# AI-Unicamp/interspeech_ser

Measured on AMD Instinct MI355X. Metric: utterances/sec (10 s @16 kHz) WavLM-large embed extract, higher is better.
Workload: dtype bf16; 1 GPU; microsoft/wavlm-large embed extract, batch=16 x 10 s @16 kHz per GPU, all 25 hidden states to HBM, mode=bf16; a counted step = 8 such batches (128 utterances per GPU), 2 in flight at a time; batch=16, batches_in_flight=2, frames_per_utt=499, parallelism=utterance-sharded x1, no collective (one process)

## Files before the change

interspeech_ser_amd/csrc/gemm.hip:

```cpp
#include "ser_common.h"
#include "launch_plan.h"
#ifndef SER_GEMM_PP
#define SER_GEMM_PP 27
#endif
#include <stdlib.h>
#include <stdio.h>
#include <utility>
#ifdef SER_GEMM_DBG
extern "C" { void* ser_gemm_dbg_ptr = nullptr; }
__device__ unsigned long long* ser_gemm_dbg_dev = nullptr;
#endif

typedef const __attribute__((address_space(1))) void* gptr_t;
typedef __attribute__((address_space(3))) void* lptr_t;

__device__ __forceinline__ const char* uniform_ptr(const void* p) {
    const uint64_t v = (uint64_t)p;
    const uint32_t lo = __builtin_amdgcn_readfirstlane((uint32_t)v), hi = __builtin_amdgcn_readfirstlane((uint32_t)(v >> 32));
    return (const char*)(((uint64_t)hi << 32) | lo);
}
template <int BYTES>
__device__ __forceinline__ void dma_lds(const void* ubase, uint32_t voff, uint32_t lds_addr) {
    static_assert(BYTES == 16 || BYTES == 4, "dwordx4 or dword");
    if constexpr (BYTES == 16)
        asm volatile("s_mov_b32 m0, %2\n\tglobal_load_lds_dwordx4 %0, %1" :: "v"(voff), "s"(ubase), "s"(lds_addr) : "memory");
    else
        asm volatile("s_mov_b32 m0, %2\n\tglobal_load_lds_dword %0, %1" :: "v"(voff), "s"(ubase), "s"(lds_addr) : "memory");
}

template <int N>
__device__ __forceinline__ void wait_vmcnt() {
    if constexpr (N == 0) asm volatile("s_waitcnt vmcnt(0)" ::: "memory");
    else if constexpr (N == 1) asm volatile("s_waitcnt vmcnt(1)" ::: "memory");
    else if constexpr (N == 2) asm volatile("s_waitcnt vmcnt(2)" ::: "memory");
    else if constexpr (N == 3) asm volatile("s_waitcnt vmcnt(3)" ::: "memory");
    else if constexpr (N == 4) asm volatile("s_waitcnt vmcnt(4)" ::: "memory");
    else if constexpr (N == 5) asm volatile("s_waitcnt vmcnt(5)" ::: "memory");
    else if constexpr (N == 6) asm volatile("s_waitcnt vmcnt(6)" ::: "memory");
    else if constexpr (N == 7) asm volatile("s_waitcnt vmcnt(7)" ::: "memory");
    else if constexpr (N == 8) asm volatile("s_waitcnt vmcnt(8)" ::: "memory");
    else if constexpr (N == 10) asm volatile("s_waitcnt vmcnt(10)" ::: "memory");
    else if constexpr (N == 12) asm volatile("s_waitcnt vmcnt(12)" ::: "memory");
    else if constexpr (N == 16) asm volatile("s_waitcnt vmcnt(16)" ::: "memory");
    else static_assert(N < 0, "add a case");
}

__device__ __forceinline__ void mfma_scale8(f32x4& acc, const i32x8& a, const i32x8& b, int sa, int sb) {
    asm volatile("v_mfma_scale_f32_16x16x128_f8f6f4 %0, %1, %2, %0, %3, %4 op_sel_hi:[0,0,0]" : "+v"(acc) : "v"(a), "v"(b), "v"(sa), "v"(sb));
}
__device__ __forceinline__ void mfma_scale_drain() {
    asm volatile("s_nop 15\n\ts_nop 15\n\ts_nop 7" ::: "memory");
}

template <int WM, int WN, int TM, int TN, int BK, int ST, int MODE, bool LNEPI, int OM = MODE>
__global__ __launch_bounds__(64 * WM * WN, 2)
void ser_gemm_kernel(const ser_gemm_args p) {
    constexpr int NW = WM * WN, NT = 64 * NW;
    constexpr int BM = WM * TM * 16, BN = WN * TN * 16;
    constexpr int CH = BK / 8;
    constexpr int ROWB = BK * 2;
    constexpr int RPP = 1024 / ROWB;
    constexpr bool M16 = (MODE == SER_MODE_FP16M);
    constexpr int NPL = M16 ? 1 : mode_traits<MODE>::planes;
    constexpr int A_BYTES = BM * ROWB, W_BYTES = BN * ROWB, STAGE = NPL * (A_BYTES + W_BYTES);
    static_assert(!M16 || (BK == 64 && !LNEPI && (BM + BN) % 64 == 0), "FP16M: 64-deep K tiles, dense epilogue");
    constexpr int SCW = BM + BN;
    constexpr int LA = BM / RPP / NW, LW = BN / RPP / NW;
    constexpr int LPT = NPL * (LA + LW);
    constexpr int KS = BK / 32;
    static_assert(BM % (RPP * NW) == 0 && BN % (RPP * NW) == 0, "tile/wave mismatch");
    extern __shared__ __attribute__((aligned(16))) char lds[];

    const int tid = threadIdx.x;
    const int lane = tid & 63;
    const int wave = __builtin_amdgcn_readfirstlane(tid >> 6);
    const int wm = wave / WN, wn = wave % WN;
#ifdef SER_GEMM_DBG
    const unsigned long long dbg_e0 = __builtin_amdgcn_s_memtime();
#endif

    const int ntn = (p.N + BN - 1) / BN;
    const int ntm = (p.M + BM - 1) / BM;
    int bid = blockIdx.x;
    {
        const int nwg = ntm * ntn;
        const int q = nwg >> 3, r = nwg & 7, xcd = bid & 7;
        const int base = (xcd < r) ? xcd * (q + 1) : r * (q + 1) + (xcd - r) * q;
        bid = base + (bid >> 3);
    }
    const int mt = bid / ntn;
    const int nt = bid - mt * ntn;
    const int g = blockIdx.y;
    const int m0 = mt * BM, n0 = nt * BN;

    const unsigned short* Abase = (const unsigned short*)p.A + (int64_t)g * p.a_group_stride;
    const unsigned short* Wbase = (const unsigned short*)p.W + (int64_t)g * p.w_group_stride;

    const int prow = lane / CH, ppos = lane % CH;
    uint32_t aoff[LA], woff[LW];
    const int m0c = m0 < p.M ? m0 : p.M - 1;
    const int64_t arow0 = p.a_rowoff ? (int64_t)p.a_rowoff[m0c] * 8 : (int64_t)m0c * p.lda;
    const char* const Atile = uniform_ptr(Abase + arow0);
    const char* const Wtile = uniform_ptr(Wbase + (int64_t)n0 * p.K);
#pragma unroll
    for (int q = 0; q < LA; ++q) {
        const int R = (q * NW + wave) * RPP + prow;
        const int f = (BK == 64) ? (R & 7) : ((R >> 1) & 3);
        const int c = ppos ^ f;
        int m = m0 + R;
        m = m < p.M ? m : p.M - 1;
        const int64_t arow = p.a_rowoff ? (int64_t)p.a_rowoff[m] * 8 : (int64_t)m * p.lda;
        aoff[q] = (uint32_t)((arow - arow0 + c * 8) * 2);
    }
#pragma unroll
    for (int q = 0; q < LW; ++q) {
        const int R = (q * NW + wave) * RPP + prow;
        const int f = (BK == 64) ? (R & 7) : ((R >> 1) & 3);
        const int c = ppos ^ f;
        int n = n0 + R;
        n = n < p.N ? n : p.N - 1;
        woff[q] = (uint32_t)(((int64_t)(n - n0) * p.K + c * 8) * 2);
    }
    const uint32_t lds0 = __builtin_amdgcn_readfirstlane((uint32_t)(uintptr_t)(__attribute__((address_space(3))) char*)lds);

    const int nk = p.K / BK;
    const int total = M16 ? 2 * nk : nk;
    const int tpc = p.kc ? p.kc / BK : 0x7fffffff;

    unsigned char* const scl = (unsigned char*)(lds + ST * STAGE + (LNEPI ? 0 : BM * 8));
    const int sc_chunk = M16 ? (wave % (SCW / 64)) : 0;
    const bool sc_is_a = sc_chunk * 64 < BM;
    const char* const sc_base = uniform_ptr(sc_is_a ? p.a_scale : p.w_scale);
    const int64_t sc_step = (sc_is_a ? p.a_scale_ld : p.w_scale_ld) * 4;
    uint32_t sc_off = 0;
    if constexpr (M16) {
        const int r = sc_chunk * 64 + lane;
        int i = sc_is_a ? m0 + r : n0 + r - BM;
        const int lim = sc_is_a ? p.M : p.N;
        i = i < lim ? i : lim - 1;
        sc_off = (uint32_t)i * 4u;
    }
    int i_kk = 0, i_cc = 0, i_cj = 0, i_stage = 0;
    const char* is_ua = nullptr; const char* is_uw = nullptr;
    uint32_t is_dstA = 0, is_dstW = 0;
    auto issue_begin = [&]() {
        int64_t koffA = (int64_t)i_cj * p.ldj + (int64_t)i_cc * BK;
        int64_t koffW = (int64_t)i_kk * BK;
        if constexpr (M16) {
            koffA = (int64_t)(i_kk >> 1) * BK + (i_kk & 1) * p.a_plane_stride;
            koffW = (int64_t)(i_kk >> 1) * BK + (i_kk & 1) * p.w_plane_stride;
            if (i_kk & 1) dma_lds<4>(sc_base + (int64_t)(i_kk >> 1) * sc_step, sc_off, lds0 + (uint32_t)(ST * STAGE + (LNEPI ? 0 : BM * 8) + (i_stage * SCW + sc_chunk * 64) * 4));
        }
        is_dstA = lds0 + i_stage * STAGE + wave * 1024;
        is_dstW = is_dstA + NPL * A_BYTES;
        is_ua = Atile + koffA * 2;
        is_uw = Wtile + koffW * 2;
    };
    auto issue_piece = [&](int j) {
        const int pl = j / (LA + LW), q = j % (LA + LW);
        if (q < LA) dma_lds<16>(is_ua + (int64_t)pl * p.a_plane_stride * 2, aoff[q < LA ? q : 0], is_dstA + pl * A_BYTES + q * NW * 1024);
        else dma_lds<16>(is_uw + (int64_t)pl * p.w_plane_stride * 2, woff[q >= LA ? q - LA : 0], is_dstW + pl * W_BYTES + (q - LA) * NW * 1024);
    };
    auto issue_end = [&]() {
        ++i_kk; ++i_cc;
        if (i_cc == tpc) { i_cc = 0; ++i_cj; }
        i_stage = (i_stage + 1 == ST) ? 0 : i_stage + 1;
    };
    auto issue = [&]() {
        issue_begin();
#pragma unroll
        for (int j = 0; j < LPT; ++j) issue_piece(j);
        issue_end();
    };

    f32x4 acc[TN][TM];
#pragma unroll
    for (int a = 0; a < TN; ++a)
#pragma unroll
        for (int b = 0; b < TM; ++b) acc[a][b] = (f32x4){0.f, 0.f, 0.f, 0.f};

    const int frow = lane & 15, fq = lane >> 4;
    const int fsw = (BK == 64) ? (lane & 7) : ((frow >> 1) & 3);
    int offA[KS], offW[KS];
#pragma unroll
    for (int s = 0; s < KS; ++s) {
        const int phys = ((s * 4 + fq) ^ fsw) << 4;
        offA[s] = (wm * TM * 16 + frow) * ROWB + phys;
        offW[s] = NPL * A_BYTES + (wn * TN * 16 + frow) * ROWB + phys;
    }

    constexpr int CPL = TN * 4;
    const int ncol0 = n0 + wn * (TN * 16) + fq * 4;
    const int64_t gcol = (int64_t)g * p.c_group_stride + ncol0;
    float bias[CPL], csum[CPL];
    auto load_cols = [&]() {
#pragma unroll
        for (int j = 0; j < CPL; ++j) { bias[j] = 0.f; csum[j] = 0.f; }
        if (p.bias) {
#pragma unroll
            for (int j4 = 0; j4 < TN; ++j4)
                if (ncol0 + j4 * 16 < p.N) {
                    const f32x4 b = *(const f32x4*)(p.bias + (int64_t)g * p.N + ncol0 + j4 * 16);
                    bias[j4 * 4 + 0] = b[0]; bias[j4 * 4 + 1] = b[1]; bias[j4 * 4 + 2] = b[2]; bias[j4 * 4 + 3] = b[3];
                }
        }
        if (p.ln_colsum) {
#pragma unroll
            for (int j4 = 0; j4 < TN; ++j4)
                if (ncol0 + j4 * 16 < p.N) {
                    const f32x4 b = *(const f32x4*)(p.ln_colsum + ncol0 + j4 * 16);
                    csum[j4 * 4 + 0] = b[0]; csum[j4 * 4 + 1] = b[1]; csum[j4 * 4 + 2] = b[2]; csum[j4 * 4 + 3] = b[3];
                }
        }
    };
    constexpr bool LATE_COLS = M16;
    if constexpr (!LATE_COLS) load_cols();

#pragma unroll
    for (int t = 0; t < ST - 1; ++t)
        if (t < total) issue();

    float* lnst = (float*)(lds + ST * STAGE);
    if (p.ln_stats_in) {
        for (int r = tid; r < BM; r += NT) {
            int m = m0 + r;
            m = m < p.M ? m : p.M - 1;
            const float* ps = p.ln_stats_in + (int64_t)m * p.ln_groups * 2;
            f32x4 pv[16];
#pragma unroll
            for (int u = 0; u < 16; ++u)
                pv[u] = (2 * u < p.ln_groups) ? *(const f32x4*)(ps + 4 * u) : (f32x4){0.f, 0.f, 0.f, 0.f};
            float s1 = 0.f, s2 = 0.f;
#pragma unroll
            for (int u = 0; u < 16; ++u) { s1 += pv[u][0] + pv[u][2]; s2 += pv[u][1] + pv[u][3]; }
            const float invK = 1.0f / (float)p.K;
            const float mu = s1 * invK;
            const float var = fmaxf(s2 * invK - mu * mu, 0.f);
            lnst[2 * r] = mu;
            lnst[2 * r + 1] = rsqrtf(var + p.ln_eps);
            if (p.mean_out && nt == 0 && g == 0 && m0 + r < p.M) p.mean_out[m] = mu + (p.ln_shift ? p.ln_shift[m] : 0.f);
            if (p.lnstat_out && nt == 0 && g == 0 && m0 + r < p.M) *(f32x2*)(p.lnstat_out + 2 * (int64_t)m) = (f32x2){mu, lnst[2 * r + 1]};
        }
        __syncthreads();
    }

#ifdef SER_GEMM_DBG
    const unsigned long long dbg_t0 = __builtin_amdgcn_s_memtime(), dbg_r0 = __builtin_amdgcn_s_memrealtime();
#endif
    constexpr int PP_BIT = NPL == 2 ? (LNEPI ? 16 : 8) : (LNEPI ? 4 : (TM * TN >= 32 ? 1 : 2));
    constexpr bool PP = !M16 && (SER_GEMM_PP & PP_BIT) && NW == 8 && (KS == 2 || NPL == 2);
    constexpr int PH = (NPL == 1 && TM * TN >= 32) ? KS : 1;
    constexpr int SPP = KS / PH;
    constexpr bool PPW = PP && NPL == 2 && KS == 1 && TN >= 8;
    if constexpr (PPW) {
        constexpr int TNH = TN / 2;
        const int late = wave >> 2;
        if (total >= ST - 1) wait_vmcnt<LPT * (ST - 2)>(); else wait_vmcnt<0>();
        __builtin_amdgcn_s_barrier();
        __builtin_amdgcn_sched_barrier(0);
        if (late) __builtin_amdgcn_s_barrier();
        int stage = 0;
        for (int kt = 0; kt < total; ++kt) {
            const bool more = kt + ST - 1 < total;
            if (more) issue();
            const char* sb = lds + stage * STAGE;
            stage = (stage + 1 == ST) ? 0 : stage + 1;
            const bool last = kt + 1 == total;
            bf16x8 ah[TM], al[TM];
#pragma unroll
            for (int ph = 0; ph < 2; ++ph) {
                bf16x8 wh[TNH], wl[TNH];
                if (ph == 0) {
#pragma unroll
                    for (int x = 0; x < TM; ++x) {
                        ah[x] = *(const bf16x8*)(sb + offA[0] + x * 16 * ROWB);
                        al[x] = *(const bf16x8*)(sb + offA[0] + A_BYTES + x * 16 * ROWB);
                    }
                }
#pragma unroll
                for (int x = 0; x < TNH; ++x) {
                    wh[x] = *(const bf16x8*)(sb + offW[0] + (ph * TNH + x) * 16 * ROWB);
                    wl[x] = *(const bf16x8*)(sb + offW[0] + W_BYTES + (ph * TNH + x) * 16 * ROWB);
                }
                asm volatile("s_waitcnt lgkmcnt(0)" ::: "memory");
                if (ph == 1 && late) { if (more) wait_vmcnt<LPT * (ST - 2)>(); else wait_vmcnt<0>(); }
                __builtin_amdgcn_sched_barrier(0);
                __builtin_amdgcn_s_barrier();
                __builtin_amdgcn_sched_barrier(0);
                __builtin_amdgcn_s_setprio(1);
#pragma unroll
                for (int nj = 0; nj < TNH; ++nj)
#pragma unroll
                    for (int mi = 0; mi < TM; ++mi) {
                        const int ni = ph * TNH + nj;
                        acc[ni][mi] = mfma16<MODE>(wl[nj], ah[mi], acc[ni][mi]);
                        acc[ni][mi] = mfma16<MODE>(wh[nj], al[mi], acc[ni][mi]);
                        acc[ni][mi] = mfma16<MODE>(wh[nj], ah[mi], acc[ni][mi]);
                    }
                __builtin_amdgcn_s_setprio(0);
                if (ph == 1 && !late) { if (more) wait_vmcnt<LPT * (ST - 2)>(); else wait_vmcnt<0>(); }
                __builtin_amdgcn_sched_barrier(0);
                if (!(ph == 1 && last && late)) __builtin_amdgcn_s_barrier();
                __builtin_amdgcn_sched_barrier(0);
            }
        }
    }
    if constexpr (PP && !PPW) {
        const int late = wave >> 2;
        if (total >= ST - 1) wait_vmcnt<LPT * (ST - 2)>(); else wait_vmcnt<0>();
        __builtin_amdgcn_s_barrier();
        __builtin_amdgcn_sched_barrier(0);
        if (late) __builtin_amdgcn_s_barrier();
        int stage = 0;
        for (int kt = 0; kt < total; ++kt) {
            const bool more = kt + ST - 1 < total;
            if (more) issue();
            const char* sb = lds + stage * STAGE;
            stage = (stage + 1 == ST) ? 0 : stage + 1;
            const bool last = kt + 1 == total;
#pragma unroll
            for (int ph = 0; ph < PH; ++ph) {
                bf16x8 af[SPP][TM], wf[SPP][TN];
                bf16x8 al[NPL == 2 ? SPP : 1][NPL == 2 ? TM : 1], wl[NPL == 2 ? SPP : 1][NPL == 2 ? TN : 1];
#pragma unroll
                for (int u = 0; u < SPP; ++u) {
#pragma unroll
                    for (int x = 0; x < TM; ++x) {
                        af[u][x] = *(const bf16x8*)(sb + offA[ph * SPP + u] + x * 16 * ROWB);
                        if constexpr (NPL == 2) al[u][x] = *(const bf16x8*)(sb + offA[ph * SPP + u] + A_BYTES + x * 16 * ROWB);
                    }
#pragma unroll
                    for (int x = 0; x < TN; ++x) {
                        wf[u][x] = *(const bf16x8*)(sb + offW[ph * SPP + u] + x * 16 * ROWB);
                        if constexpr (NPL == 2) wl[u][x] = *(const bf16x8*)(sb + offW[ph * SPP + u] + W_BYTES + x * 16 * ROWB);
                    }
                }
                asm volatile("s_waitcnt lgkmcnt(0)" ::: "memory");
                if (ph == PH - 1 && late) { if (more) wait_vmcnt<LPT * (ST - 2)>(); else wait_vmcnt<0>(); }
                __builtin_amdgcn_sched_barrier(0);
                __builtin_amdgcn_s_barrier();
                __builtin_amdgcn_sched_barrier(0);
                __builtin_amdgcn_s_setprio(1);
#pragma unroll
                for (int u = 0; u < SPP; ++u)
#pragma unroll
                    for (int ni = 0; ni < TN; ++ni)
#pragma unroll
                        for (int mi = 0; mi < TM; ++mi) {
                            if constexpr (NPL == 2) {
                                acc[ni][mi] = mfma16<MODE>(wl[u][ni], af[u][mi], acc[ni][mi]);
                                acc[ni][mi] = mfma16<MODE>(wf[u][ni], al[u][mi], acc[ni][mi]);
                                acc[ni][mi] = mfma16<MODE>(wf[u][ni], af[u][mi], acc[ni][mi]);
                            } else {
                                acc[ni][mi] = mfma16<MODE>(wf[u][ni], af[u][mi], acc[ni][mi]);
                            }
                        }
                __builtin_amdgcn_s_setprio(0);
                if (ph == PH - 1 && !late) { if (more) wait_vmcnt<LPT * (ST - 2)>(); else wait_vmcnt<0>(); }
                __builtin_amdgcn_sched_barrier(0);
                if (!(ph == PH - 1 && last && late)) __builtin_amdgcn_s_barrier();
                __builtin_amdgcn_sched_barrier(0);
            }
        }
    }

    if constexpr (M16) {
        constexpr int LPTH = LPT, LPTE = LPT + 1;
        constexpr bool PPM = (NW == 8);
        constexpr int PHM = (TM * TN >= 32) ? 2 : 1;
        constexpr int SPM = KS / PHM;
        constexpr int PHE = PHM;
        constexpr int TMP = TM / PHE;
        auto wait_landed = [&](bool more, int young) {
            if (!more || ST == 2) wait_vmcnt<0>();
            else if (young & 1) wait_vmcnt<LPTE * (ST - 2)>();
            else wait_vmcnt<LPTH * (ST - 2)>();
        };
        auto h_phase_reads = [&](const char* sb, int ph, auto& af, auto& wf) {
#pragma unroll
            for (int u = 0; u < SPM; ++u) {
#pragma unroll
                for (int x = 0; x < TM; ++x) af[u][x] = *(const bf16x8*)(sb + offA[ph * SPM + u] + x * 16 * ROWB);
#pragma unroll
                for (int x = 0; x < TN; ++x) wf[u][x] = *(const bf16x8*)(sb + offW[ph * SPM + u] + x * 16 * ROWB);
            }
        };
        auto h_phase_mfma = [&](auto& af, auto& wf) {
#pragma unroll
            for (int u = 0; u < SPM; ++u)
#pragma unroll
                for (int ni = 0; ni < TN; ++ni)
#pragma unroll
                    for (int mi = 0; mi < TM; ++mi) acc[ni][mi] = mfma16<SER_MODE_FP16>(wf[u][ni], af[u][mi], acc[ni][mi]);
        };
        auto e_phase_reads = [&](const char* sb, const unsigned char* scb, int ph, auto& a8, auto& w8, auto& sa, auto& sw) {
#pragma unroll
            for (int x = 0; x < TMP; ++x) {
                const int mi = ph * TMP + x;
                const u32x4 c0 = *(const u32x4*)(sb + offA[0] + mi * 16 * ROWB), c1 = *(const u32x4*)(sb + offA[1] + mi * 16 * ROWB);
                a8[x] = (i32x8){(int)c0[0], (int)c0[1], (int)c0[2], (int)c0[3], (int)c1[0], (int)c1[1], (int)c1[2], (int)c1[3]};
                sa[x] = scb[(wm * TM * 16 + mi * 16 + frow) * 4 + fq];
            }
#pragma unroll
            for (int x = 0; x < TN; ++x) {
                const u32x4 c0 = *(const u32x4*)(sb + offW[0] + x * 16 * ROWB), c1 = *(const u32x4*)(sb + offW[1] + x * 16 * ROWB);
                w8[x] = (i32x8){(int)c0[0], (int)c0[1], (int)c0[2], (int)c0[3], (int)c1[0], (int)c1[1], (int)c1[2], (int)c1[3]};
                sw[x] = scb[(BM + wn * TN * 16 + x * 16 + frow) * 4 + fq];
            }
        };
        auto e_phase_mfma = [&](int ph, auto& a8, auto& w8, auto& sa, auto& sw) {
#pragma unroll
            for (int ni = 0; ni < TN; ++ni)
#pragma unroll
                for (int x = 0; x < TMP; ++x)
                    mfma_scale8(acc[ni][ph * TMP + x], w8[ni], a8[x], sw[ni], sa[x]);
        };
        if constexpr (PPM) {
            const int late = wave >> 2;
            wait_landed(total >= ST - 1, ST - 2);
            __builtin_amdgcn_s_barrier();
            __builtin_amdgcn_sched_barrier(0);
            if (late) __builtin_amdgcn_s_barrier();
            int stage = 0;
            auto unit = [&](int kt, auto etag) {
                constexpr bool EU = decltype(etag)::value;
                const bool more = kt + ST - 1 < total;
#ifdef SER_GEMM_DBG
                unsigned long long stp[8] = {0, 0, 0, 0, 0, 0, 0, 0};
                const bool stamp = ser_gemm_dbg_dev && blockIdx.x == 40 && lane == 0 && kt >= 8 && kt < 16;
#define SER_STAMP(i) do { __builtin_amdgcn_sched_barrier(0); if (stamp) stp[i] = __builtin_amdgcn_s_memtime(); __builtin_amdgcn_sched_barrier(0); } while (0)
                SER_STAMP(0);
#else
#define SER_STAMP(i) do { } while (0)
#endif
                SER_STAMP(1);
                const char* sb = lds + stage * STAGE;
                const unsigned char* scb = scl + stage * SCW * 4;
                stage = (stage + 1 == ST) ? 0 : stage + 1;
                const bool last = kt + 1 == total;
                constexpr int NPH = EU ? PHE : PHM;
#pragma unroll
                for (int ph = 0; ph < NPH; ++ph) {
                    bf16x8 af[EU ? 1 : SPM][EU ? 1 : TM], wf[EU ? 1 : SPM][EU ? 1 : TN];
                    i32x8 a8[EU ? TMP : 1], w8[EU ? TN : 1];
                    int sa[EU ? TMP : 1], sw[EU ? TN : 1];
                    if constexpr (!EU) h_phase_reads(sb, ph, af, wf);
                    else e_phase_reads(sb, scb, ph, a8, w8, sa, sw);
                    if (ph == 0 && more) { __builtin_amdgcn_sched_barrier(0); issue(); }
                    asm volatile("s_waitcnt lgkmcnt(0)" ::: "memory");
                    if (ph == 0) SER_STAMP(2);
                    if (ph == NPH - 1 && late) wait_landed(more, kt + ST - 1);
                    if (ph == 0) SER_STAMP(3);
                    __builtin_amdgcn_sched_barrier(0);
                    __builtin_amdgcn_s_barrier();
                    __builtin_amdgcn_sched_barrier(0);
                    if (ph == 0) SER_STAMP(4);
                    __builtin_amdgcn_s_setprio(1);
                    if constexpr (!EU) h_phase_mfma(af, wf);
                    else e_phase_mfma(ph, a8, w8, sa, sw);
                    __builtin_amdgcn_s_setprio(0);
                    if (ph == 0) SER_STAMP(5);
                    if (ph == NPH - 1 && !late) wait_landed(more, kt + ST - 1);
                    if (ph == 0) SER_STAMP(6);
                    __builtin_amdgcn_sched_barrier(0);
                    if (!(ph == NPH - 1 && last && late)) __builtin_amdgcn_s_barrier();
                    __builtin_amdgcn_sched_barrier(0);
                    if (ph == 0) SER_STAMP(7);
                }
#ifdef SER_GEMM_DBG
                if (stamp) for (int i = 0; i < 8; ++i) ser_gemm_dbg_dev[262144 + ((wave * 8 + (kt - 8)) * 8 + i)] = stp[i];
#endif
            };
            for (int kt = 0; kt < total; kt += 2) {
                unit(kt, std::false_type{});
                unit(kt + 1, std::true_type{});
            }
        } else {
            int stage = 0;
            auto unit = [&](int kt, auto etag) {
                constexpr bool EU = decltype(etag)::value;
                wait_landed(kt + (ST - 2) < total, kt + ST - 2);
                __builtin_amdgcn_s_barrier();
                if (kt + ST - 1 < total) issue();
                const char* sb = lds + stage * STAGE;
                const unsigned char* scb = scl + stage * SCW * 4;
                stage = (stage + 1 == ST) ? 0 : stage + 1;
#pragma unroll
                for (int ph = 0; ph < (EU ? PHE : PHM); ++ph) {
                    if constexpr (!EU) {
                        bf16x8 af[SPM][TM], wf[SPM][TN];
                        h_phase_reads(sb, ph, af, wf);
                        __builtin_amdgcn_s_setprio(1);
                        h_phase_mfma(af, wf);
                        __builtin_amdgcn_s_setprio(0);
                    } else {
                        i32x8 a8[TMP], w8[TN];
                        int sa[TMP], sw[TN];
                        e_phase_reads(sb, scb, ph, a8, w8, sa, sw);
                        __builtin_amdgcn_s_setprio(1);
                        e_phase_mfma(ph, a8, w8, sa, sw);
                        __builtin_amdgcn_s_setprio(0);
                    }
                }
            };
            for (int kt = 0; kt < total; kt += 2) {
                unit(kt, std::false_type{});
                unit(kt + 1, std::true_type{});
            }
        }
    }
    if constexpr (M16) mfma_scale_drain();
    int c_stage = 0;
    for (int kt = 0; kt < ((PP || M16) ? 0 : total); ++kt) {
        if (kt + (ST - 2) < total) wait_vmcnt<LPT * (ST - 2)>();
        else wait_vmcnt<0>();
        __builtin_amdgcn_s_barrier();
        if (kt + ST - 1 < total) issue();
        const char* sb = lds + c_stage * STAGE;
        c_stage = (c_stage + 1 == ST) ? 0 : c_stage + 1;
        if constexpr (NPL == 1) {
            constexpr bool PIPE = (TM * TN * 4 + KS * (TM + TN) * 4) <= 208;
            bf16x8 af[KS][TM], wf[KS][TN];
            if constexpr (PIPE) {
#pragma unroll
                for (int s = 0; s < KS; ++s) {
#pragma unroll
                    for (int x = 0; x < TM; ++x) af[s][x] = *(const bf16x8*)(sb + offA[s] + x * 16 * ROWB);
#pragma unroll
                    for (int x = 0; x < TN; ++x) wf[s][x] = *(const bf16x8*)(sb + offW[s] + x * 16 * ROWB);
                }
            }
#pragma unroll
            for (int s = 0; s < KS; ++s) {
                if constexpr (!PIPE) {
#pragma unroll
                    for (int x = 0; x < TM; ++x) af[s][x] = *(const bf16x8*)(sb + offA[s] + x * 16 * ROWB);
#pragma unroll
                    for (int x = 0; x < TN; ++x) wf[s][x] = *(const bf16x8*)(sb + offW[s] + x * 16 * ROWB);
                }
                __builtin_amdgcn_s_setprio(1);
#pragma unroll
                for (int ni = 0; ni < TN; ++ni)
#pragma unroll
                    for (int mi = 0; mi < TM; ++mi)
                        acc[ni][mi] = mfma16<MODE>(wf[s][ni], af[s][mi], acc[ni][mi]);
                __builtin_amdgcn_s_setprio(0);
            }
        } else {
#pragma unroll
            for (int s = 0; s < KS; ++s) {
                bf16x8 ah[TM], al[TM], wh[TN], wl[TN];
#pragma unroll
                for (int x = 0; x < TM; ++x) {
                    ah[x] = *(const bf16x8*)(sb + offA[s] + x * 16 * ROWB);
                    al[x] = *(const bf16x8*)(sb + offA[s] + A_BYTES + x * 16 * ROWB);
                }
#pragma unroll
                for (int x = 0; x < TN; ++x) {
                    wh[x] = *(const bf16x8*)(sb + offW[s] + x * 16 * ROWB);
                    wl[x] = *(const bf16x8*)(sb + offW[s] + W_BYTES + x * 16 * ROWB);
                }
                __builtin_amdgcn_s_setprio(1);
#pragma unroll
                for (int ni = 0; ni < TN; ++ni)
#pragma unroll
                    for (int mi = 0; mi < TM; ++mi) {
                        acc[ni][mi] = mfma16<MODE>(wl[ni], ah[mi], acc[ni][mi]);
                        acc[ni][mi] = mfma16<MODE>(wh[ni], al[mi], acc[ni][mi]);
                        acc[ni][mi] = mfma16<MODE>(wh[ni], ah[mi], acc[ni][mi]);
                    }
                __builtin_amdgcn_s_setprio(0);
            }
        }
    }

#ifdef SER_GEMM_DBG
    {
        __builtin_amdgcn_sched_barrier(0);
        const unsigned long long t1 = __builtin_amdgcn_s_memtime(), r1 = __builtin_amdgcn_s_memrealtime();
        unsigned long long* d = ser_gemm_dbg_dev;
        if (d && wave == 0 && lane == 0 && blockIdx.y == 0) {
            d[blockIdx.x * 2] = t1 - dbg_t0; d[blockIdx.x * 2 + 1] = r1 - dbg_r0;
            d[131072 + blockIdx.x * 4] = dbg_t0 - dbg_e0; d[131072 + blockIdx.x * 4 + 1] = t1;
        }
    }
#endif
    if constexpr (LATE_COLS) load_cols();
    float ramax = 0.f;
    if constexpr (LNEPI) {
        __syncthreads();
        float* red = (float*)lds;
        const float invN = 1.0f / (float)p.N;
        float mean[TM], rstd[TM], nmr[TM];
#pragma unroll
        for (int mi = 0; mi < TM; ++mi) {
            float s1 = 0.f, s2 = 0.f;
#pragma unroll
            for (int ni = 0; ni < TN; ++ni)
#pragma unroll
                for (int r = 0; r < 4; ++r) {
                    const float x = acc[ni][mi][r] + bias[ni * 4 + r];
                    acc[ni][mi][r] = x;
                    if (ncol0 + ni * 16 < p.N) { s1 += x; s2 += x * x; }
                }
            s1 += __shfl_xor(s1, 16, 64); s2 += __shfl_xor(s2, 16, 64);
            s1 += __shfl_xor(s1, 32, 64); s2 += __shfl_xor(s2, 32, 64);
            if (fq == 0) {
                red[((wm * TM * 16 + mi * 16 + frow) * WN + wn) * 2] = s1;
                red[((wm * TM * 16 + mi * 16 + frow) * WN + wn) * 2 + 1] = s2;
            }
        }
        __syncthreads();
#pragma unroll
        for (int mi = 0; mi < TM; ++mi) {
            float s1 = 0.f, s2 = 0.f;
#pragma unroll
            for (int w = 0; w < WN; ++w) {
                s1 += red[((wm * TM * 16 + mi * 16 + frow) * WN + w) * 2];
                s2 += red[((wm * TM * 16 + mi * 16 + frow) * WN + w) * 2 + 1];
            }
            mean[mi] = s1 * invN;
            rstd[mi] = rsqrtf(fmaxf(s2 * invN - mean[mi] * mean[mi], 0.f) + p.ln_eps);
            nmr[mi] = -mean[mi] * rstd[mi];
        }
        float lg[CPL], lb[CPL];
#pragma unroll
        for (int j4 = 0; j4 < TN; ++j4) {
            f32x4 a = {0.f, 0.f, 0.f, 0.f}, b = {0.f, 0.f, 0.f, 0.f};
            if (ncol0 + j4 * 16 < p.N) {
                a = *(const f32x4*)(p.ln_gamma + ncol0 + j4 * 16);
                b = *(const f32x4*)(p.ln_beta + ncol0 + j4 * 16);
            }
#pragma unroll
            for (int r = 0; r < 4; ++r) { lg[j4 * 4 + r] = a[r]; lb[j4 * 4 + r] = b[r]; }
        }
#pragma unroll
        for (int mi = 0; mi < TM; ++mi) {
            const int m = m0 + wm * TM * 16 + mi * 16 + frow;
            if (m >= p.M) continue;
            const int64_t orow = p.out_rowmap ? (int64_t)p.out_rowmap[m] : (int64_t)m;
#pragma unroll
            for (int ni = 0; ni < TN; ni += 2) {
                const bool ok0 = ncol0 + ni * 16 < p.N, ok1 = ncol0 + ni * 16 + 16 < p.N;
                float v[8];
#pragma unroll
                for (int r = 0; r < 8; ++r) {
                    const int nj = ni + (r >> 2), rr = r & 3;
                    v[r] = fmaf(fmaf(acc[nj][mi][rr], rstd[mi], nmr[mi]), lg[nj * 4 + rr], lb[nj * 4 + rr]);
                }
                if (p.act == SER_ACT_GELU) {
#pragma unroll
                    for (int r = 0; r < 8; r += 2) {
                        const f32x2 y = gelu2<MODE == SER_MODE_BF16>((f32x2){v[r], v[r + 1]});
                        v[r] = y[0]; v[r + 1] = y[1];
                    }
                }
                if (p.out_f32) {
                    f32x4 o0 = {v[0], v[1], v[2], v[3]}, o1 = {v[4], v[5], v[6], v[7]};
                    if (ok0) *(f32x4*)(p.out_f32 + (int64_t)m * p.ldo_f32 + gcol + ni * 16) = o0;
                    if (ok1) *(f32x4*)(p.out_f32 + (int64_t)m * p.ldo_f32 + gcol + ni * 16 + 16) = o1;
                }
                if (p.out_act) {
                    const int c8 = ni * 16 + ((fq & 1) ? 12 : 0);
                    store_act8_swap<MODE>((unsigned short*)p.out_act + orow * p.ldo_act + gcol + c8, p.out_plane_stride,
                                          ncol0 + c8 < p.N, v);
                    if constexpr (mode_traits<MODE>::f16) {
                        if (p.range_flag) range_fold8(ramax, v, ok0, ok1);
                    }
                }
            }
        }
    } else {
        const bool do_scale = p.col_scale_end > 0;
        const bool do_stat = p.stat_out != nullptr;
        float cs[TM];
#pragma unroll
        for (int mi = 0; mi < TM; ++mi) {
            cs[mi] = 0.f;
            if (p.shift_out) {
                int m = m0 + wm * TM * 16 + mi * 16 + frow;
                m = m < p.M ? m : p.M - 1;
                cs[mi] = p.shift_const + (p.shift_in ? p.shift_in[m] : 0.f);
            }
        }
        constexpr int RB = (TM * TN > 16) ? 2 : (TM < 4 ? TM : 4);
        f32x4 rres[RB][TN];
#pragma unroll
        for (int mi = 0; mi < TM; ++mi) {
            if (mi % RB == 0 && p.residual) {
#pragma unroll
                for (int u = 0; u < RB; ++u) {
                    int mr = m0 + wm * TM * 16 + (mi + u) * 16 + frow;
                    mr = mr < p.M ? mr : p.M - 1;
                    const int rr_ = p.res_row_mod ? (mr % p.res_row_mod) : mr;
#pragma unroll
                    for (int ni = 0; ni < TN; ++ni) {
                        f32x4 r = {0.f, 0.f, 0.f, 0.f};
                        if (ncol0 + ni * 16 < p.N) r = *(const f32x4*)(p.residual + (int64_t)rr_ * p.ldr + gcol + ni * 16);
                        rres[u][ni] = r;
                    }
                }
            }
            const int m = m0 + wm * TM * 16 + mi * 16 + frow;
            if (m >= p.M) continue;
            const int64_t orow = p.out_rowmap ? (int64_t)p.out_rowmap[m] : (int64_t)m;
            float mu = 0.f, rs = 1.f;
            if (p.ln_stats_in) {
                mu = lnst[2 * (wm * TM * 16 + mi * 16 + frow)];
                rs = lnst[2 * (wm * TM * 16 + mi * 16 + frow) + 1];
            }
            const float cshift = cs[mi];
            if (p.shift_out && nt == 0 && g == 0 && wn == 0 && fq == 0) p.shift_out[m] = cshift;
            const float* gsc = nullptr;
            const float* gsh = nullptr;
            if (p.gn_scale) {
                int lo = 0, hi = p.gn_B;
                while (hi - lo > 1) { const int mid = (lo + hi) >> 1; if (p.gn_row_offs[mid] <= m) lo = mid; else hi = mid; }
                gsc = p.gn_scale + (int64_t)lo * p.gn_ld + ncol0;
                gsh = p.gn_shift + (int64_t)lo * p.gn_ld + ncol0;
            }
            float st1 = 0.f, st2 = 0.f;
            unsigned mcode[2] = {0u, 0u};
#pragma unroll
            for (int ni = 0; ni < TN; ni += 2) {
                const bool ok0 = ncol0 + ni * 16 < p.N, ok1 = ncol0 + ni * 16 + 16 < p.N;
                float v[8];
#pragma unroll
                for (int r = 0; r < 8; ++r) {
                    const int nj = ni + (r >> 2), rr = r & 3;
                    float x = fmaf(rs, acc[nj][mi][rr] - mu * csum[nj * 4 + rr], bias[nj * 4 + rr]);
                    if (gsc && ncol0 + nj * 16 < p.N) x = fmaf(x, gsc[nj * 16 + rr], gsh[nj * 16 + rr]);
                    if (do_scale && ncol0 + nj * 16 < p.col_scale_end) x *= p.col_scale;
                    v[r] = x;
                }
                if (p.act == SER_ACT_GELU) {
#pragma unroll
                    for (int r = 0; r < 8; r += 2) {
                        const f32x2 y = gelu2<MODE == SER_MODE_BF16>((f32x2){v[r], v[r + 1]});
                        v[r] = y[0]; v[r + 1] = y[1];
                    }
                }
                if (p.residual) {
                    const f32x4 r0 = rres[mi % RB][ni], r1 = rres[mi % RB][ni + 1];
                    v[0] += r0[0]; v[1] += r0[1]; v[2] += r0[2]; v[3] += r0[3];
                    v[4] += r1[0]; v[5] += r1[1]; v[6] += r1[2]; v[7] += r1[3];
                }
                if (p.out_f32) {
                    float* op = p.out_f32 + (int64_t)m * p.ldo_f32 + gcol + ni * 16 - p.f32_col_begin;
                    f32x4 o0 = {v[0], v[1], v[2], v[3]}, o1 = {v[4], v[5], v[6], v[7]};
                    if (ok0 && ncol0 + ni * 16 >= p.f32_col_begin) *(f32x4*)op = o0;
                    if (ok1 && ncol0 + ni * 16 + 16 >= p.f32_col_begin) *(f32x4*)(op + 16) = o1;
                }
                if (p.shift_out) {
#pragma unroll
                    for (int r = 0; r < 8; ++r) v[r] -= cshift;
                }
                if (do_stat && ok0) {
#pragma unroll
                    for (int r = 0; r < 4; ++r) { st1 += v[r]; st2 += v[r] * v[r]; }
                }
                if (do_stat && ok1) {
#pragma unroll
                    for (int r = 4; r < 8; ++r) { st1 += v[r]; st2 += v[r] * v[r]; }
                }
                if (p.out_act) {
                    const int c8 = ni * 16 + ((fq & 1) ? 12 : 0);
                    if constexpr (OM == SER_MODE_FP16M) {
                        store_act8_swap<SER_MODE_FP16>((unsigned short*)p.out_act + orow * p.ldo_act + gcol + c8, 0, ncol0 + c8 < p.N, v);
                        float lo[8], ax = 0.f, al = 0.f;
#pragma unroll
                        for (int r = 0; r < 8; r += 2) {
                            const unsigned h2 = pack_h2(v[r], v[r + 1]);
                            lo[r] = v[r] - h2f((unsigned short)(h2 & 0xffffu));
                            lo[r + 1] = v[r + 1] - h2f((unsigned short)(h2 >> 16));
                            ax = fmaxf(ax, fmaxf(fabsf(v[r]), fabsf(v[r + 1])));
                            al = fmaxf(al, fmaxf(fabsf(lo[r]), fabsf(lo[r + 1])));
                        }
                        if (p.range_flag) range_fold8(ramax, v, ok0, ok1);
                        ax = max_rowquad(ax); al = max_rowquad(al);
                        const unsigned cx = mx_code(ax), cl = mx_code(al);
                        const float ix = mx_inv(cx), il = mx_inv(cl);
                        unsigned q4[4] = {mx_pack4(lo[0] * il, lo[1] * il, lo[2] * il, lo[3] * il), mx_pack4(lo[4] * il, lo[5] * il, lo[6] * il, lo[7] * il),
                                          mx_pack4(v[0] * ix, v[1] * ix, v[2] * ix, v[3] * ix), mx_pack4(v[4] * ix, v[5] * ix, v[6] * ix, v[7] * ix)};
                        transpose_rowquad(q4);
                        const int64_t bcol = gcol - fq * 4 + ni * 16;
                        unsigned char* seg = (unsigned char*)((unsigned short*)p.out_act + p.out_plane_stride) + (orow * p.ldo_act + (bcol & ~(int64_t)63)) * 2;
                        if (ok0) *(u32x4*)(seg + (fq >> 1) * 64 + (bcol & 63) + (fq & 1) * 16) = (u32x4){q4[0], q4[1], q4[2], q4[3]};
                        mcode[(ni >> 1) & 1] = cl | (cx << 16);
                        if (((ni >> 1) & 1) && fq == 0 && ok0)
                            p.out_scale[(bcol >> 6) * p.out_scale_ld + orow] = (mcode[0] & 0xffu) | ((mcode[1] & 0xffu) << 8) | (mcode[0] & 0xff0000u) | ((mcode[1] & 0xff0000u) << 8);
                    } else {
                        store_act8_swap<OM>((unsigned short*)p.out_act + orow * p.ldo_act + gcol + c8, p.out_plane_stride,
                                            ncol0 + c8 < p.N, v);
                        if constexpr (mode_traits<OM>::f16) {
                            if (p.range_flag) range_fold8(ramax, v, ok0, ok1);
                        }
                    }
                }
            }
            if (p.stat_out) {
                st1 += __shfl_xor(st1, 16, 64); st2 += __shfl_xor(st2, 16, 64);
                st1 += __shfl_xor(st1, 32, 64); st2 += __shfl_xor(st2, 32, 64);
                const int cstart = n0 + wn * (TN * 16);
                const int grp = g * ((p.N + 63) >> 6) + (cstart >> 6);
                if (fq == 0 && cstart < p.N && grp < p.stat_groups) {
                    float* d = p.stat_out + ((int64_t)m * p.stat_groups + grp) * 2;
                    d[0] = st1; d[1] = st2;
                    if constexpr (TN * 16 > 64) {
                        if (cstart + 64 < p.N) { d[2] = 0.f; d[3] = 0.f; }
                    }
                }
            }
        }
    }
    if constexpr (mode_traits<OM>::f16) range_report(p.range_flag, ramax);
#ifdef SER_GEMM_DBG
    {
        __builtin_amdgcn_sched_barrier(0);
        asm volatile("s_waitcnt vmcnt(0)" ::: "memory");
        const unsigned long long t2 = __builtin_amdgcn_s_memtime();
        unsigned long long* d = ser_gemm_dbg_dev;
        if (d && wave == 0 && lane == 0 && blockIdx.y == 0) d[131072 + blockIdx.x * 4 + 2] = t2;
    }
#endif
}

template <int... I, class F>
static bool with_index(int i, std::integer_sequence<int, I...>, F&& f) { return ser_with_mode<I...>(i, f); }

template <int TILE, int PAIR>
static int launch_planned(const ser_gemm_args* a, const gemm_launch& pl, hipStream_t s) {
    constexpr gemm_tile t = GEMM_TILE[TILE];
    constexpr gemm_pair pr = GEMM_PAIR[PAIR];
    auto k = ser_gemm_kernel<t.WM, t.WN, t.TM, t.TN, t.BK, t.ST, pr.mode, t.LNEPI, pr.om>;
    static std::atomic<bool> ready{false};
    if (pl.lds > 65536)
        if (hipError_t e = ser_lds_optin(k, pl.lds, ready)) return ser_fail((int)e, "ser_gemm: cannot raise dynamic LDS to %d", pl.lds);
    hipLaunchKernelGGL(k, dim3(pl.grid_x, pl.grid_y, 1), dim3((unsigned)pl.block, 1, 1), pl.lds, s, *a);
    return ser_check_launch("ser_gemm");
}

extern "C" int ser_gemm(const ser_gemm_args* a, void* stream) {
    gemm_launch pl;
    if (int rc = gemm_plan(a, &pl)) return rc;
// ... 20 lines not shown
```

Baseline: 2061 utterances/s.

## Skip dead M-tail fragments in GEMM main loops and epilogues

Computes a per-wave count of live 16-row fragments and, for tail tiles, runs a specialized K-loop that skips LDS reads and MFMAs for rows beyond M. Epilogue, LN-stat and residual loops also break early past the live rows, and LN stat rows past M are filled with defaults instead of clamped reloads. The change targets wasted matrix work in the partial last M tile (frames_per_utt=499 makes M non-aligned). In exchange it doubles the instantiated loop bodies, which costs code size and could raise register pressure, and it is excluded for several configurations through TAIL_RULE.

```diff
diff --git a/interspeech_ser_amd/csrc/gemm.hip b/interspeech_ser_amd/csrc/gemm.hip
--- a/interspeech_ser_amd/csrc/gemm.hip
+++ b/interspeech_ser_amd/csrc/gemm.hip
@@ -50,6 +50,37 @@
 }
 __device__ __forceinline__ void mfma_scale_drain() {
     asm volatile("s_nop 15\n\ts_nop 15\n\ts_nop 7" ::: "memory");
+}
+
+template <int TM, class F>
+__device__ __forceinline__ void frag_rows(bool full, int lv, F&& f) {
+#pragma unroll
+    for (int mi = 0; mi < TM; ++mi) {
+        if (!full && mi >= lv) break;
+        f(mi);
+    }
+}
+template <int TN, int TM, class F>
+__device__ __forceinline__ void frag_pairs(bool full, int lv, F&& f) {
+    if (full) {
+#pragma unroll
+        for (int ni = 0; ni < TN; ++ni)
+#pragma unroll
+            for (int mi = 0; mi < TM; ++mi) f(ni, mi);
+    } else {
+#pragma unroll
+        for (int mi = 0; mi < TM; ++mi) {
+            if (mi >= lv) break;
+#pragma unroll
+            for (int ni = 0; ni < TN; ++ni) f(ni, mi);
+        }
+    }
+}
+template <int TM>
+__device__ __forceinline__ int live_rows(bool full, int live) {
+    if (full) return TM;
+    asm volatile("" : "+s"(live));
+    return live;
 }
 
 template <int WM, int WN, int TM, int TN, int BK, int ST, int MODE, bool LNEPI, int OM = MODE>
@@ -92,6 +123,12 @@
     const int nt = bid - mt * ntn;
     const int g = blockIdx.y;
     const int m0 = mt * BM, n0 = nt * BN;
+    constexpr bool TAIL_RULE = !((NPL == 2 && TN == 8) || (NPL == 1 && LNEPI && WM == 2) || (NPL == 2 && OM == SER_MODE_FP16M) ||
+                                 (NPL == 2 && BK == 64 && MODE == SER_MODE_FP16X && OM == SER_MODE_FP16X) ||
+                                 (MODE == SER_MODE_FP16 && OM == SER_MODE_FP16X && TM * TN == 32));
+    const int live = TAIL_RULE ? __builtin_amdgcn_readfirstlane(max(0, min(TM, (p.M - m0 - wm * TM * 16 + 15) >> 4))) : TM;
+    using full_k = std::true_type;
+    using tail_k = std::false_type;
 
     const unsigned short* Abase = (const unsigned short*)p.A + (int64_t)g * p.a_group_stride;
     const unsigned short* Wbase = (const unsigned short*)p.W + (int64_t)g * p.w_group_stride;
@@ -223,8 +260,8 @@
     float* lnst = (float*)(lds + ST * STAGE);
     if (p.ln_stats_in) {
         for (int r = tid; r < BM; r += NT) {
-            int m = m0 + r;
-            m = m < p.M ? m : p.M - 1;
+            const int m = m0 + r;
+            if (m >= p.M) { lnst[2 * r] = 0.f; lnst[2 * r + 1] = 1.f; continue; }
             const float* ps = p.ln_stats_in + (int64_t)m * p.ln_groups * 2;
             f32x4 pv[16];
 #pragma unroll
@@ -238,8 +275,8 @@
             const float var = fmaxf(s2 * invK - mu * mu, 0.f);
             lnst[2 * r] = mu;
             lnst[2 * r + 1] = rsqrtf(var + p.ln_eps);
-            if (p.mean_out && nt == 0 && g == 0 && m0 + r < p.M) p.mean_out[m] = mu + (p.ln_shift ? p.ln_shift[m] : 0.f);
-            if (p.lnstat_out && nt == 0 && g == 0 && m0 + r < p.M) *(f32x2*)(p.lnstat_out + 2 * (int64_t)m) = (f32x2){mu, lnst[2 * r + 1]};
+            if (p.mean_out && nt == 0 && g == 0) p.mean_out[m] = mu + (p.ln_shift ? p.ln_shift[m] : 0.f);
+            if (p.lnstat_out && nt == 0 && g == 0) *(f32x2*)(p.lnstat_out + 2 * (int64_t)m) = (f32x2){mu, lnst[2 * r + 1]};
         }
         __syncthreads();
     }
@@ -312,6 +349,8 @@
         __builtin_amdgcn_sched_barrier(0);
         if (late) __builtin_amdgcn_s_barrier();
         int stage = 0;
+        auto kloop = [&](auto kform) {
+        constexpr bool FULL = decltype(kform)::value;
         for (int kt = 0; kt < total; ++kt) {
             const bool more = kt + ST - 1 < total;
             if (more) issue();
@@ -320,19 +359,21 @@
             const bool last = kt + 1 == total;
 #pragma unroll
             for (int ph = 0; ph < PH; ++ph) {
+                const int lv = live_rows<TM>(FULL, live);
                 bf16x8 af[SPP][TM], wf[SPP][TN];
                 bf16x8 al[NPL == 2 ? SPP : 1][NPL == 2 ? TM : 1], wl[NPL == 2 ? SPP : 1][NPL == 2 ? TN : 1];
 #pragma unroll
                 for (int u = 0; u < SPP; ++u) {
-#pragma unroll
-                    for (int x = 0; x < TM; ++x) {
+                    frag_rows<TM>(FULL, lv, [&](int x) {
                         af[u][x] = *(const bf16x8*)(sb + offA[ph * SPP + u] + x * 16 * ROWB);
                         if constexpr (NPL == 2) al[u][x] = *(const bf16x8*)(sb + offA[ph * SPP + u] + A_BYTES + x * 16 * ROWB);
-                    }
-#pragma unroll
-                    for (int x = 0; x < TN; ++x) {
-                        wf[u][x] = *(const bf16x8*)(sb + offW[ph * SPP + u] + x * 16 * ROWB);
-                        if constexpr (NPL == 2) wl[u][x] = *(const bf16x8*)(sb + offW[ph * SPP + u] + W_BYTES + x * 16 * ROWB);
+                    });
+                    if (FULL || lv > 0) {
+#pragma unroll
+                        for (int x = 0; x < TN; ++x) {
+                            wf[u][x] = *(const bf16x8*)(sb + offW[ph * SPP + u] + x * 16 * ROWB);
+                            if constexpr (NPL == 2) wl[u][x] = *(const bf16x8*)(sb + offW[ph * SPP + u] + W_BYTES + x * 16 * ROWB);
+                        }
                     }
                 }
                 asm volatile("s_waitcnt lgkmcnt(0)" ::: "memory");
@@ -343,18 +384,15 @@
                 __builtin_amdgcn_s_setprio(1);
 #pragma unroll
                 for (int u = 0; u < SPP; ++u)
-#pragma unroll
-                    for (int ni = 0; ni < TN; ++ni)
-#pragma unroll
-                        for (int mi = 0; mi < TM; ++mi) {
-                            if constexpr (NPL == 2) {
-                                acc[ni][mi] = mfma16<MODE>(wl[u][ni], af[u][mi], acc[ni][mi]);
-                                acc[ni][mi] = mfma16<MODE>(wf[u][ni], al[u][mi], acc[ni][mi]);
-                                acc[ni][mi] = mfma16<MODE>(wf[u][ni], af[u][mi], acc[ni][mi]);
-                            } else {
-                                acc[ni][mi] = mfma16<MODE>(wf[u][ni], af[u][mi], acc[ni][mi]);
-                            }
+                    frag_pairs<TN, TM>(FULL, lv, [&](int ni, int mi) {
+                        if constexpr (NPL == 2) {
+                            acc[ni][mi] = mfma16<MODE>(wl[u][ni], af[u][mi], acc[ni][mi]);
+                            acc[ni][mi] = mfma16<MODE>(wf[u][ni], al[u][mi], acc[ni][mi]);
+                            acc[ni][mi] = mfma16<MODE>(wf[u][ni], af[u][mi], acc[ni][mi]);
+                        } else {
+                            acc[ni][mi] = mfma16<MODE>(wf[u][ni], af[u][mi], acc[ni][mi]);
                         }
+                    });
                 __builtin_amdgcn_s_setprio(0);
                 if (ph == PH - 1 && !late) { if (more) wait_vmcnt<LPT * (ST - 2)>(); else wait_vmcnt<0>(); }
                 __builtin_amdgcn_sched_barrier(0);
@@ -362,6 +400,8 @@
                 __builtin_amdgcn_sched_barrier(0);
             }
         }
+        };
+        if (live == TM) kloop(full_k{}); else kloop(tail_k{});
     }
 
     if constexpr (M16) {
@@ -376,44 +416,50 @@
             else if (young & 1) wait_vmcnt<LPTE * (ST - 2)>();
             else wait_vmcnt<LPTH * (ST - 2)>();
         };
-        auto h_phase_reads = [&](const char* sb, int ph, auto& af, auto& wf) {
+        auto h_phase_reads = [&](const char* sb, int ph, int lv, auto& af, auto& wf) {
 #pragma unroll
             for (int u = 0; u < SPM; ++u) {
 #pragma unroll
-                for (int x = 0; x < TM; ++x) af[u][x] = *(const bf16x8*)(sb + offA[ph * SPM + u] + x * 16 * ROWB);
-#pragma unroll
-                for (int x = 0; x < TN; ++x) wf[u][x] = *(const bf16x8*)(sb + offW[ph * SPM + u] + x * 16 * ROWB);
+                for (int x = 0; x < TM; ++x)
+                    if (x < lv) af[u][x] = *(const bf16x8*)(sb + offA[ph * SPM + u] + x * 16 * ROWB);
+#pragma unroll
+                for (int x = 0; x < TN; ++x)
+                    if (lv > 0) wf[u][x] = *(const bf16x8*)(sb + offW[ph * SPM + u] + x * 16 * ROWB);
             }
         };
-        auto h_phase_mfma = [&](auto& af, auto& wf) {
+        auto h_phase_mfma = [&](int lv, auto& af, auto& wf) {
 #pragma unroll
             for (int u = 0; u < SPM; ++u)
 #pragma unroll
                 for (int ni = 0; ni < TN; ++ni)
 #pragma unroll
-                    for (int mi = 0; mi < TM; ++mi) acc[ni][mi] = mfma16<SER_MODE_FP16>(wf[u][ni], af[u][mi], acc[ni][mi]);
+                    for (int mi = 0; mi < TM; ++mi)
+                        if (mi < lv) acc[ni][mi] = mfma16<SER_MODE_FP16>(wf[u][ni], af[u][mi], acc[ni][mi]);
         };
-        auto e_phase_reads = [&](const char* sb, const unsigned char* scb, int ph, auto& a8, auto& w8, auto& sa, auto& sw) {
+        auto e_phase_reads = [&](const char* sb, const unsigned char* scb, int ph, int lv, auto& a8, auto& w8, auto& sa, auto& sw) {
 #pragma unroll
             for (int x = 0; x < TMP; ++x) {
                 const int mi = ph * TMP + x;
-                const u32x4 c0 = *(const u32x4*)(sb + offA[0] + mi * 16 * ROWB), c1 = *(const u32x4*)(sb + offA[1] + mi * 16 * ROWB);
-                a8[x] = (i32x8){(int)c0[0], (int)c0[1], (int)c0[2], (int)c0[3], (int)c1[0], (int)c1[1], (int)c1[2], (int)c1[3]};
-                sa[x] = scb[(wm * TM * 16 + mi * 16 + frow) * 4 + fq];
-            }
-#pragma unroll
-            for (int x = 0; x < TN; ++x) {
-                const u32x4 c0 = *(const u32x4*)(sb + offW[0] + x * 16 * ROWB), c1 = *(const u32x4*)(sb + offW[1] + x * 16 * ROWB);
-                w8[x] = (i32x8){(int)c0[0], (int)c0[1], (int)c0[2], (int)c0[3], (int)c1[0], (int)c1[1], (int)c1[2], (int)c1[3]};
-                sw[x] = scb[(BM + wn * TN * 16 + x * 16 + frow) * 4 + fq];
-            }
+                if (mi < lv) {
+                    const u32x4 c0 = *(const u32x4*)(sb + offA[0] + mi * 16 * ROWB), c1 = *(const u32x4*)(sb + offA[1] + mi * 16 * ROWB);
+                    a8[x] = (i32x8){(int)c0[0], (int)c0[1], (int)c0[2], (int)c0[3], (int)c1[0], (int)c1[1], (int)c1[2], (int)c1[3]};
+                    sa[x] = scb[(wm * TM * 16 + mi * 16 + frow) * 4 + fq];
+                }
+            }
+#pragma unroll
+            for (int x = 0; x < TN; ++x)
+                if (ph * TMP < lv) {
+                    const u32x4 c0 = *(const u32x4*)(sb + offW[0] + x * 16 * ROWB), c1 = *(const u32x4*)(sb + offW[1] + x * 16 * ROWB);
+                    w8[x] = (i32x8){(int)c0[0], (int)c0[1], (int)c0[2], (int)c0[3], (int)c1[0], (int)c1[1], (int)c1[2], (int)c1[3]};
+                    sw[x] = scb[(BM + wn * TN * 16 + x * 16 + frow) * 4 + fq];
+                }
         };
-        auto e_phase_mfma = [&](int ph, auto& a8, auto& w8, auto& sa, auto& sw) {
+        auto e_phase_mfma = [&](int ph, int lv, auto& a8, auto& w8, auto& sa, auto& sw) {
 #pragma unroll
             for (int ni = 0; ni < TN; ++ni)
 #pragma unroll
                 for (int x = 0; x < TMP; ++x)
-                    mfma_scale8(acc[ni][ph * TMP + x], w8[ni], a8[x], sw[ni], sa[x]);
+                    if (ph * TMP + x < lv) mfma_scale8(acc[ni][ph * TMP + x], w8[ni], a8[x], sw[ni], sa[x]);
         };
         if constexpr (PPM) {
             const int late = wave >> 2;
@@ -422,8 +468,9 @@
             __builtin_amdgcn_sched_barrier(0);
             if (late) __builtin_amdgcn_s_barrier();
             int stage = 0;
-            auto unit = [&](int kt, auto etag) {
+            auto unit = [&](int kt, auto etag, auto kform) {
                 constexpr bool EU = decltype(etag)::value;
+                const int lv = live_rows<TM>(decltype(kform)::value, live);
                 const bool more = kt + ST - 1 < total;
 #ifdef SER_GEMM_DBG
                 unsigned long long stp[8] = {0, 0, 0, 0, 0, 0, 0, 0};
@@ -444,8 +491,8 @@
                     bf16x8 af[EU ? 1 : SPM][EU ? 1 : TM], wf[EU ? 1 : SPM][EU ? 1 : TN];
                     i32x8 a8[EU ? TMP : 1], w8[EU ? TN : 1];
                     int sa[EU ? TMP : 1], sw[EU ? TN : 1];
-                    if constexpr (!EU) h_phase_reads(sb, ph, af, wf);
-                    else e_phase_reads(sb, scb, ph, a8, w8, sa, sw);
+                    if constexpr (!EU) h_phase_reads(sb, ph, lv, af, wf);
+                    else e_phase_reads(sb, scb, ph, lv, a8, w8, sa, sw);
                     if (ph == 0 && more) { __builtin_amdgcn_sched_barrier(0); issue(); }
                     asm volatile("s_waitcnt lgkmcnt(0)" ::: "memory");
                     if (ph == 0) SER_STAMP(2);
@@ -456,8 +503,8 @@
                     __builtin_amdgcn_sched_barrier(0);
                     if (ph == 0) SER_STAMP(4);
                     __builtin_amdgcn_s_setprio(1);
-                    if constexpr (!EU) h_phase_mfma(af, wf);
-                    else e_phase_mfma(ph, a8, w8, sa, sw);
+                    if constexpr (!EU) h_phase_mfma(lv, af, wf);
+                    else e_phase_mfma(ph, lv, a8, w8, sa, sw);
                     __builtin_amdgcn_s_setprio(0);
                     if (ph == 0) SER_STAMP(5);
                     if (ph == NPH - 1 && !late) wait_landed(more, kt + ST - 1);
@@ -471,14 +518,18 @@
                 if (stamp) for (int i = 0; i < 8; ++i) ser_gemm_dbg_dev[262144 + ((wave * 8 + (kt - 8)) * 8 + i)] = stp[i];
 #endif
             };
-            for (int kt = 0; kt < total; kt += 2) {
-                unit(kt, std::false_type{});
-                unit(kt + 1, std::true_type{});
-            }
+            auto kloop = [&](auto kform) {
+                for (int kt = 0; kt < total; kt += 2) {
+                    unit(kt, std::false_type{}, kform);
+                    unit(kt + 1, std::true_type{}, kform);
+                }
+            };
+            if (live == TM) kloop(full_k{}); else kloop(tail_k{});
         } else {
             int stage = 0;
-            auto unit = [&](int kt, auto etag) {
+            auto unit = [&](int kt, auto etag, auto kform) {
                 constexpr bool EU = decltype(etag)::value;
+                const int lv = live_rows<TM>(decltype(kform)::value, live);
                 wait_landed(kt + (ST - 2) < total, kt + ST - 2);
                 __builtin_amdgcn_s_barrier();
                 if (kt + ST - 1 < total) issue();
@@ -489,29 +540,35 @@
                 for (int ph = 0; ph < (EU ? PHE : PHM); ++ph) {
                     if constexpr (!EU) {
                         bf16x8 af[SPM][TM], wf[SPM][TN];
-                        h_phase_reads(sb, ph, af, wf);
+                        h_phase_reads(sb, ph, lv, af, wf);
                         __builtin_amdgcn_s_setprio(1);
-                        h_phase_mfma(af, wf);
+                        h_phase_mfma(lv, af, wf);
                         __builtin_amdgcn_s_setprio(0);
                     } else {
                         i32x8 a8[TMP], w8[TN];
                         int sa[TMP], sw[TN];
-                        e_phase_reads(sb, scb, ph, a8, w8, sa, sw);
+                        e_phase_reads(sb, scb, ph, lv, a8, w8, sa, sw);
                         __builtin_amdgcn_s_setprio(1);
-                        e_phase_mfma(ph, a8, w8, sa, sw);
+                        e_phase_mfma(ph, lv, a8, w8, sa, sw);
                         __builtin_amdgcn_s_setprio(0);
                     }
                 }
             };
-            for (int kt = 0; kt < total; kt += 2) {
-                unit(kt, std::false_type{});
-                unit(kt + 1, std::true_type{});
-            }
+            auto kloop = [&](auto kform) {
+                for (int kt = 0; kt < total; kt += 2) {
+                    unit(kt, std::false_type{}, kform);
+                    unit(kt + 1, std::true_type{}, kform);
+                }
+            };
+            if (live == TM) kloop(full_k{}); else kloop(tail_k{});
         }
     }
     if constexpr (M16) mfma_scale_drain();
     int c_stage = 0;
+    auto ring = [&](auto kform) {
+    constexpr bool FULL = decltype(kform)::value;
     for (int kt = 0; kt < ((PP || M16) ? 0 : total); ++kt) {
+        const int lv = live_rows<TM>(FULL, live);
         if (kt + (ST - 2) < total) wait_vmcnt<LPT * (ST - 2)>();
         else wait_vmcnt<0>();
         __builtin_amdgcn_s_barrier();
@@ -525,25 +582,25 @@
 #pragma unroll
                 for (int s = 0; s < KS; ++s) {
 #pragma unroll
-                    for (int x = 0; x < TM; ++x) af[s][x] = *(const bf16x8*)(sb + offA[s] + x * 16 * ROWB);
-#pragma unroll
-                    for (int x = 0; x < TN; ++x) wf[s][x] = *(const bf16x8*)(sb + offW[s] + x * 16 * ROWB);
+                    for (int x = 0; x < TM; ++x)
+                        if (FULL || x < lv) af[s][x] = *(const bf16x8*)(sb + offA[s] + x * 16 * ROWB);
+#pragma unroll
+                    for (int x = 0; x < TN; ++x)
+                        if (FULL || lv > 0) wf[s][x] = *(const bf16x8*)(sb + offW[s] + x * 16 * ROWB);
                 }
             }
 #pragma unroll
             for (int s = 0; s < KS; ++s) {
                 if constexpr (!PIPE) {
 #pragma unroll
-                    for (int x = 0; x < TM; ++x) af[s][x] = *(const bf16x8*)(sb + offA[s] + x * 16 * ROWB);
-#pragma unroll
-                    for (int x = 0; x < TN; ++x) wf[s][x] = *(const bf16x8*)(sb + offW[s] + x * 16 * ROWB);
+                    for (int x = 0; x < TM; ++x)
+                        if (FULL || x < lv) af[s][x] = *(const bf16x8*)(sb + offA[s] + x * 16 * ROWB);
+#pragma unroll
+                    for (int x = 0; x < TN; ++x)
+                        if (FULL || lv > 0) wf[s][x] = *(const bf16x8*)(sb + offW[s] + x * 16 * ROWB);
                 }
                 __builtin_amdgcn_s_setprio(1);
-#pragma unroll
-                for (int ni = 0; ni < TN; ++ni)
-#pragma unroll
-                    for (int mi = 0; mi < TM; ++mi)
-                        acc[ni][mi] = mfma16<MODE>(wf[s][ni], af[s][mi], acc[ni][mi]);
+                frag_pairs<TN, TM>(FULL, lv, [&](int ni, int mi) { acc[ni][mi] = mfma16<MODE>(wf[s][ni], af[s][mi], acc[ni][mi]); });
                 __builtin_amdgcn_s_setprio(0);
             }
         } else {
@@ -551,28 +608,29 @@
             for (int s = 0; s < KS; ++s) {
                 bf16x8 ah[TM], al[TM], wh[TN], wl[TN];
 #pragma unroll
-                for (int x = 0; x < TM; ++x) {
-                    ah[x] = *(const bf16x8*)(sb + offA[s] + x * 16 * ROWB);
-                    al[x] = *(const bf16x8*)(sb + offA[s] + A_BYTES + x * 16 * ROWB);
-                }
-#pragma unroll
-                for (int x = 0; x < TN; ++x) {
-                    wh[x] = *(const bf16x8*)(sb + offW[s] + x * 16 * ROWB);
-                    wl[x] = *(const bf16x8*)(sb + offW[s] + W_BYTES + x * 16 * ROWB);
-                }
+                for (int x = 0; x < TM; ++x)
+                    if (FULL || x < lv) {
+                        ah[x] = *(const bf16x8*)(sb + offA[s] + x * 16 * ROWB);
+                        al[x] = *(const bf16x8*)(sb + offA[s] + A_BYTES + x * 16 * ROWB);
+                    }
+#pragma unroll
+                for (int x = 0; x < TN; ++x)
+                    if (FULL || lv > 0) {
+                        wh[x] = *(const bf16x8*)(sb + offW[s] + x * 16 * ROWB);
+                        wl[x] = *(const bf16x8*)(sb + offW[s] + W_BYTES + x * 16 * ROWB);
+                    }
                 __builtin_amdgcn_s_setprio(1);
-#pragma unroll
-                for (int ni = 0; ni < TN; ++ni)
-#pragma unroll
-                    for (int mi = 0; mi < TM; ++mi) {
-                        acc[ni][mi] = mfma16<MODE>(wl[ni], ah[mi], acc[ni][mi]);
-                        acc[ni][mi] = mfma16<MODE>(wh[ni], al[mi], acc[ni][mi]);
-                        acc[ni][mi] = mfma16<MODE>(wh[ni], ah[mi], acc[ni][mi]);
-                    }
+                frag_pairs<TN, TM>(FULL, lv, [&](int ni, int mi) {
+                    acc[ni][mi] = mfma16<MODE>(wl[ni], ah[mi], acc[ni][mi]);
+                    acc[ni][mi] = mfma16<MODE>(wh[ni], al[mi], acc[ni][mi]);
+                    acc[ni][mi] = mfma16<MODE>(wh[ni], ah[mi], acc[ni][mi]);
+                });
                 __builtin_amdgcn_s_setprio(0);
             }
         }
     }
+    };
+    if constexpr (!PP && !M16) { if (live == TM) ring(full_k{}); else ring(tail_k{}); }
 
 #ifdef SER_GEMM_DBG
     {
@@ -595,6 +653,7 @@
 #pragma unroll
         for (int mi = 0; mi < TM; ++mi) {
             float s1 = 0.f, s2 = 0.f;
+            if (mi < live) {
 #pragma unroll
             for (int ni = 0; ni < TN; ++ni)
 #pragma unroll
@@ -605,6 +664,7 @@
                 }
             s1 += __shfl_xor(s1, 16, 64); s2 += __shfl_xor(s2, 16, 64);
             s1 += __shfl_xor(s1, 32, 64); s2 += __shfl_xor(s2, 32, 64);
+            }
             if (fq == 0) {
                 red[((wm * TM * 16 + mi * 16 + frow) * WN + wn) * 2] = s1;
                 red[((wm * TM * 16 + mi * 16 + frow) * WN + wn) * 2 + 1] = s2;
@@ -613,6 +673,7 @@
         __syncthreads();
 #pragma unroll
         for (int mi = 0; mi < TM; ++mi) {
+            if (mi >= live) break;
             float s1 = 0.f, s2 = 0.f;
 #pragma unroll
             for (int w = 0; w < WN; ++w) {
@@ -636,6 +697,7 @@
         }
 #pragma unroll
         for (int mi = 0; mi < TM; ++mi) {
+            if (mi >= live) break;
             const int m = m0 + wm * TM * 16 + mi * 16 + frow;
             if (m >= p.M) continue;
             const int64_t orow = p.out_rowmap ? (int64_t)p.out_rowmap[m] : (int64_t)m;
@@ -677,7 +739,7 @@
 #pragma unroll
         for (int mi = 0; mi < TM; ++mi) {
             cs[mi] = 0.f;
-            if (p.shift_out) {
+            if (p.shift_out && mi < live) {
                 int m = m0 + wm * TM * 16 + mi * 16 + frow;
                 m = m < p.M ? m : p.M - 1;
                 cs[mi] = p.shift_const + (p.shift_in ? p.shift_in[m] : 0.f);
@@ -687,9 +749,11 @@
         f32x4 rres[RB][TN];
 #pragma unroll
         for (int mi = 0; mi < TM; ++mi) {
+            if (mi >= live) break;
             if (mi % RB == 0 && p.residual) {
 #pragma unroll
                 for (int u = 0; u < RB; ++u) {
+                    if (mi + u >= live) break;
                     int mr = m0 + wm * TM * 16 + (mi + u) * 16 + frow;
                     mr = mr < p.M ? mr : p.M - 1;
                     const int rr_ = p.res_row_mod ? (mr % p.res_row_mod) : mr;
```

After: 2067 utterances/s, median of 6. Within noise of the previous version (+0.3%).
